# adityamwagh/SuperSLAM

Hardware: AMD Instinct MI355X
Metric: stereo pairs/sec (SPx2+LG) at 1376x376 (higher is better)
Workload: dtype f16; 1 GPU; configs[1]: SuperPoint x2 + select + gather + 1x LightGlue on 1376x376 stereo pairs; a step = 8 x 64 = 512 pairs per GPU resident in HBM (8 library calls of 64 pairs, different images per call), max_keypoints 600, seeded synthetic weights; pairs_per_call=64, max_keypoints=600, matches_last_call=1412, parallelism=replicated weights, pairs sharded over 1 rank(s), no data-path collective

## Files before the change

### superslam_amd/csrc/api.hip

```cpp
#include <algorithm>
#include <atomic>
#include <cmath>
#include <cstdarg>
#include <cstdlib>
#include <cstring>
#include <fstream>
#include <map>
#include <memory>
#include <mutex>
#include <string>
#include <vector>

#include "../../include/sship.h"
#include "../../include/superslam_hip/place_recognizer.hpp"
#include "kernels.h"
#include "stage_layout.h"

namespace sship {

static thread_local std::string g_err;
static void (*g_log_cb)(int, const char*) = nullptr;
static int g_profiling = 0;

void set_error(const std::string& msg) {
// ... 791 lines not shown
  KpRefineArgs r{};
  r.logits = sp->logits.as<float>(); r.img_stride = (size_t)Hc * Wc * kLogitStride; r.cell_stride = kLogitStride; r.chan_stride = 1;
  r.Hc = Hc; r.Wc = Wc; r.pix = sp->pix.as<int>(); r.n_dev = n_dev; r.n_host = 0; r.max_kp = sp->cfg.max_keypoints;
  r.kp_xys = kp; r.scale_x = scale_x; r.scale_y = scale_y; r.offsets = nullptr;
  launch_kp_refine(r, B, s);
  return hipGetLastError();
}
static int sp_select(sship_sp* sp, int B, int H, int W, float* scores_out, float* kp_out, int* n_out, hipStream_t s) {
  int H2, W2, H4, W4, Hc, Wc;
  sp_shapes(H, W, H2, W2, H4, W4, Hc, Wc);
  if (sp->cand_zero_ptr != sp->cand_count.p || sp->cand_zero_n < B || sp->cand_zero_stream != s)
    SSHIP_HIP_CHECK(hipMemsetAsync(sp->cand_count.p, 0, (size_t)B * 4, s));
  sp->cand_zero_ptr = sp->cand_count.p; sp->cand_zero_n = 0; sp->cand_zero_stream = s;
  NmsArgs a{};
  a.logits = sp->logits.as<float>(); a.ls = kLogitStride; a.B = B; a.H = Hc * 8; a.W = Wc * 8;
  a.radius = sp->cfg.nms_radius; a.thr_f = sp->thr_f; a.border = sp->cfg.remove_borders;
  a.cand = sp->cand.as<unsigned long long>(); a.cand_count = sp->cand_count.as<int>(); a.cap = sp->cap;
  a.scores_out = scores_out;
  launch_nms_tile(0, a, s);
  g_timer.mark_fine("sp_extract_stereo:select/nms_tile", s);
  TopkArgs t{};
  t.cand = a.cand; t.cand_count = a.cand_count; t.cap = sp->cap; t.max_kp = sp->cfg.max_keypoints;
  t.score_w = Wc * 8;
  t.scale_x = static_cast<float>(W) / (Wc * 8);
  t.scale_y = static_cast<float>(H) / (Hc * 8);
  t.desc_h = Hc; t.desc_w = Wc; t.kp_xys = kp_out; t.cell_h = sp->cell_h.as<int>(); t.cell_w = sp->cell_w.as<int>();
  t.n_out = n_out; t.n_cand_out = nullptr; t.reset_count = a.cand_count;
  t.pix = sp_wants_pix(sp) ? sp->pix.as<int>() : nullptr;
  launch_topk(t, B, s);
  SSHIP_HIP_CHECK(hipGetLastError());
  sp->cand_zero_n = B;
  if (sp->kp_refinement == SSHIP_KP_SUBPIXEL) {
    g_timer.mark_fine("sp_extract_stereo:select/topk", s);
    SSHIP_HIP_CHECK(sp_refine(sp, B, Hc, Wc, kp_out, n_out, t.scale_x, t.scale_y, s));
    g_timer.mark(g_profiling >= 2 ? "sp_extract_stereo:select/kp_refine" : "sp_extract_stereo:select", s);
    return SSHIP_OK;
  }
  g_timer.mark(g_profiling >= 2 ? "sp_extract_stereo:select/topk" : "sp_extract_stereo:select", s);
  return SSHIP_OK;
}

static hipError_t conv1ab(sship_sp* sp, const uint8_t* img, _Float16* out, int B, int H, int W, hipStream_t s) {
#if SSHIP_DEV_SWITCHES
  if (conv_mode() == 2) return sp_conv1ab_fused(sp->c1b, sp->w1a_frag, sp->b1a, img, out, B, H, W, s);
#endif
  return sp_conv1ab_pp(sp->c1b, sp->w1a_fragb, sp->b1a, img, out, B, H, W, s);
}

extern "C" int sship_sp_create(const sship_sp_config* cfg, sship_sp** out) {
  bind_thread();
  if (!cfg || !out || !cfg->weights_path) return fail(SSHIP_ERR_INVALID, "sp_create: null argument");
  if (cfg->max_keypoints <= 0 || cfg->max_keypoints > kMaxKp) return fail(SSHIP_ERR_INVALID, "sp_create: max_keypoints must be in [1, 4096]");
  if (cfg->nms_radius < 0 || cfg->nms_radius > 8) return fail(SSHIP_ERR_INVALID, "sp_create: nms_radius must be in [0, 8]");
  if (int rc = require_device()) return rc;
  StateDict sd; std::string err;
  if (!load_safetensors(cfg->weights_path, sd, err)) return fail(SSHIP_ERR_IO, err);
  std::unique_ptr<sship_sp, void (*)(sship_sp*)> sp(new sship_sp(), sship_sp_destroy);
  sp->cfg = *cfg;
  if (sp->cfg.pool_slots <= 0) sp->cfg.pool_slots = 8;
  if (sp->cfg.max_batch <= 0) sp->cfg.max_batch = 2;
  sp->cfg.weights_path = nullptr;
  sp->thr_f = threshold_as_float(cfg->keypoint_threshold);
  struct L { const char* name; int cout, cin, ks, ct; ConvW* dst; };
  const L layers[] = {{"conv1b", 64, 64, 3, 64, &sp->c1b}, {"conv2a", 64, 64, 3, 64, &sp->c2a},
                      {"conv2b", 64, 64, 3, 64, &sp->c2b}, {"conv3a", 128, 64, 3, 64, &sp->c3a},
                      {"conv3b", 128, 128, 3, 32, &sp->c3b}, {"conv4a", 128, 128, 3, 32, &sp->c4a},
                      {"conv4b", 128, 128, 3, 32, &sp->c4b}, {"convPa", 256, 128, 3, 32, &sp->cPa},
                      {"convPb", 65, 256, 1, 96, &sp->cPb}, {"convDa", 256, 128, 3, 32, &sp->cDa},
                      {"convDb", 256, 256, 1, 128, &sp->cDb}};
  for (const L& l : layers) {
    const Tensor* w = find_tensor(sd, std::string(l.name) + ".weight", {l.cout, l.cin, l.ks, l.ks}, err);
    const Tensor* b = w ? find_tensor(sd, std::string(l.name) + ".bias", {l.cout}, err) : nullptr;
    if (!w || !b) return fail(SSHIP_ERR_IO, err);
    if (int rc = upload_conv(w->data.data(), b->data.data(), l.cout, l.cin, l.ks, l.ct, *l.dst)) return rc;
    if (l.ks == 3 && std::string(l.name) != "convDa" && std::string(l.name) != "conv1b")
      if (int rc = upload_conv_q(w->data.data(), l.cout, l.cin, *l.dst)) return rc;
#if SSHIP_DEV_SWITCHES
    if (std::string(l.name) == "conv2a" || std::string(l.name) == "conv2b")
      if (int rc = upload_wino(w->data.data(), *l.dst)) return rc;
#endif
    if (std::string(l.name) == "convDb")
      if (int rc = upload_conv(w->data.data(), b->data.data(), l.cout, l.cin, 1, 32, sp->cDb32)) return rc;
    if (std::string(l.name) == "convPb") {
      std::vector<_Float16> plain((size_t)80 * 256, (_Float16)0.f);
      for (int co = 0; co < 65; ++co)
        for (int ci = 0; ci < 256; ++ci) plain[(size_t)co * 256 + ci] = (_Float16)w->data[(size_t)co * 256 + ci];
      SSHIP_HIP_CHECK(hipMalloc(reinterpret_cast<void**>(&l.dst->w_q), plain.size() * sizeof(_Float16)));
      SSHIP_HIP_CHECK(hipMemcpy(l.dst->w_q, plain.data(), plain.size() * sizeof(_Float16), hipMemcpyHostToDevice));
    }
  }
  {
    const Tensor* w = find_tensor(sd, "conv1a.weight", {64, 1, 3, 3}, err);
    const Tensor* b = w ? find_tensor(sd, "conv1a.bias", {64}, err) : nullptr;
    if (!w || !b) return fail(SSHIP_ERR_IO, err);
    std::vector<float> wt(576);
    for (int co = 0; co < 64; ++co)
      for (int t = 0; t < 9; ++t) wt[t * 64 + co] = (float)(_Float16)w->data[co * 9 + t];
    if (int rc = upload_floats(wt.data(), 576, &sp->w1a)) return rc;
    if (int rc = upload_floats(b->data.data(), 64, &sp->b1a)) return rc;
    std::vector<_Float16> fr(2 * 64 * 8);
    for (int mt = 0; mt < 2; ++mt)
      for (int lane = 0; lane < 64; ++lane)
        for (int e = 0; e < 8; ++e) {
          const int co = mt * 32 + (lane & 31), k = (lane >> 5) * 8 + e;
          fr[(mt * 64 + lane) * 8 + e] = (_Float16)(k < 9 ? w->data[co * 9 + k] : 0.f);
        }
    SSHIP_HIP_CHECK(hipMalloc(reinterpret_cast<void**>(&sp->w1a_frag), fr.size() * sizeof(_Float16)));
    SSHIP_HIP_CHECK(hipMemcpy(sp->w1a_frag, fr.data(), fr.size() * sizeof(_Float16), hipMemcpyHostToDevice));
    std::fill(fr.begin(), fr.end(), (_Float16)0.f);
    for (int mt = 0; mt < 2; ++mt)
      for (int lane = 0; lane < 64; ++lane) {
        const int co = mt * 32 + (lane & 31), hh = lane >> 5;
        _Float16* f = &fr[(mt * 64 + lane) * 8];
        if (hh == 0) {
          for (int e = 0; e < 5; ++e) f[e] = (_Float16)w->data[co * 9 + e];
        } else {
          for (int e = 0; e < 4; ++e) f[e] = (_Float16)w->data[co * 9 + 5 + e];
          const _Float16 hi = (_Float16)b->data[co];
          f[4] = hi;
          f[5] = (_Float16)(b->data[co] - (float)hi);
        }
      }
    SSHIP_HIP_CHECK(hipMalloc(reinterpret_cast<void**>(&sp->w1a_fragb), fr.size() * sizeof(_Float16)));
    SSHIP_HIP_CHECK(hipMemcpy(sp->w1a_fragb, fr.data(), fr.size() * sizeof(_Float16), hipMemcpyHostToDevice));
  }
  SSHIP_HIP_CHECK(hipStreamCreateWithFlags(&sp->stream, hipStreamDefault));
  if (int rc = sship_pool_create(sp->cfg.pool_slots, sp->cfg.max_keypoints, SSHIP_DESC_DIM, &sp->pool)) return rc;
  *out = sp.release();
  return SSHIP_OK;
}
extern "C" void sship_sp_destroy(sship_sp* sp) {
  bind_thread();
  if (!sp) return;
  (void)hipDeviceSynchronize();
  for (ConvW* c : {&sp->c1b, &sp->c2a, &sp->c2b, &sp->c3a, &sp->c3b, &sp->c4a, &sp->c4b, &sp->cPa, &sp->cPb, &sp->cDa, &sp->cDb, &sp->cDb32})
    free_conv(*c);
  if (sp->w1a) (void)hipFree(sp->w1a);
  if (sp->b1a) (void)hipFree(sp->b1a);
  if (sp->w1a_frag) (void)hipFree(sp->w1a_frag);
  if (sp->w1a_fragb) (void)hipFree(sp->w1a_fragb);
  ring_free(sp);
  if (sp->pool) sship_pool_destroy(sp->pool);
  sp->pool = nullptr;
  if (sp->stream) (void)hipStreamDestroy(sp->stream);
  delete sp;
}
extern "C" int sship_sp_debug_activation(sship_sp* sp, int layer, void* out_host, unsigned long long bytes) {
  bind_thread();
  if (!sp || !out_host) return fail(SSHIP_ERR_INVALID, "sp_debug_activation: null argument");
  DevBuf* bufs[12] = {nullptr, &sp->a1b, &sp->a2a, &sp->a2b, &sp->a3a, &sp->a3b, &sp->a4a, &sp->a4b, &sp->aPa, &sp->aDa, &sp->draw, &sp->logits};
  if (layer < 1 || layer > 11 || !bufs[layer]->p || bytes > bufs[layer]->bytes) return fail(SSHIP_ERR_INVALID, "sp_debug_activation: bad layer / size");
  SSHIP_HIP_CHECK(hipDeviceSynchronize());
  SSHIP_HIP_CHECK(hipMemcpy(out_host, bufs[layer]->p, bytes, hipMemcpyDeviceToHost));
  return SSHIP_OK;
}
extern "C" sship_pool* sship_sp_pool(sship_sp* sp) {
  bind_thread(); return sp ? sp->pool : nullptr; }
extern "C" int sship_sp_max_keypoints(const sship_sp* sp) { return sp ? sp->cfg.max_keypoints : 0; }
extern "C" int sship_sp_set_descriptor_sampling(sship_sp* sp, int mode) {
  if (!sp) return fail(SSHIP_ERR_INVALID, "sp_set_descriptor_sampling: null handle");
  if (mode != SSHIP_DESC_NEAREST && mode != SSHIP_DESC_BILINEAR)
    return fail(SSHIP_ERR_INVALID, "sp_set_descriptor_sampling: mode must be 0 (nearest) or 1 (bilinear)");
  for (const auto& pd : sp->ring.pending)
    if (pd.active) return fail(SSHIP_ERR_INVALID, "sp_set_descriptor_sampling: a ring submission is pending (collect it with sship_sp_extract_stereo_ring first)");
#if SSHIP_DEV_SWITCHES
  if (mode == SSHIP_DESC_BILINEAR && desc_dense_mode()) return fail(SSHIP_ERR_INVALID, "sp_set_descriptor_sampling: bilinear sampling is not available under SUPERSLAM_HIP_DESC=dense");
#endif
  sp->desc_sampling = mode;
  return SSHIP_OK;
}
extern "C" int sship_sp_descriptor_sampling(const sship_sp* sp) { return sp ? sp->desc_sampling : SSHIP_DESC_NEAREST; }
extern "C" int sship_sp_set_keypoint_refinement(sship_sp* sp, int mode) {
  if (!sp) return fail(SSHIP_ERR_INVALID, "sp_set_keypoint_refinement: null handle");
  if (mode != SSHIP_KP_INTEGER && mode != SSHIP_KP_SUBPIXEL)
    return fail(SSHIP_ERR_INVALID, "sp_set_keypoint_refinement: mode must be 0 (integer) or 1 (sub-pixel)");
  for (const auto& pd : sp->ring.pending)
    if (pd.active) return fail(SSHIP_ERR_INVALID, "sp_set_keypoint_refinement: a ring submission is pending (collect it with sship_sp_extract_stereo_ring first)");
  sp->kp_refinement = mode;
  return SSHIP_OK;
}
extern "C" int sship_sp_keypoint_refinement(const sship_sp* sp) { return sp ? sp->kp_refinement : SSHIP_KP_INTEGER; }

extern "C" int sship_sp_extract_batch_device(sship_sp* sp, const uint8_t* imgs, int batch, int h, int w, void* desc_out,
                                             float* kp_out, int* n_out, void* stream) {
  bind_thread();
  if (!sp || !imgs || !desc_out || !kp_out || !n_out || batch <= 0) return fail(SSHIP_ERR_INVALID, "sp_extract_batch_device: bad arguments");
  hipStream_t s = static_cast<hipStream_t>(stream);
  if (int rc = sp_ensure(sp, batch, h, w)) return rc;
  if (g_profiling && imgs != sp->img.as<uint8_t>())
    SSHIP_HIP_CHECK(hipMemcpyAsync(sp->img.p, imgs, (size_t)batch * h * w, hipMemcpyDeviceToDevice, s));
  sp->img_valid = g_profiling != 0 || imgs == sp->img.as<uint8_t>();
  g_timer.begin(s);
  if (int rc = sp_network(sp, imgs, batch, h, w, s, false)) return rc;
  if (int rc = sp_select(sp, batch, h, w, nullptr, kp_out, n_out, s)) return rc;
  int H2, W2, H4, W4, Hc, Wc;
  sp_shapes(h, w, H2, W2, H4, W4, Hc, Wc);
  SSHIP_HIP_CHECK(desc_head(sp, 0, Hc, Wc, sp->cell_h.as<int>(), sp->cell_w.as<int>(), n_out, batch, static_cast<_Float16*>(desc_out),
                            (size_t)sp->cfg.max_keypoints * 256, s));
  g_timer.mark("sp_extract_stereo:gather", s);
  return SSHIP_OK;
}

extern "C" int sship_sp_dense(sship_sp* sp, const uint8_t* imgs, int batch, int h, int w, float* scores, void* desc_grid,
                              float* logits, void* stream) {
  bind_thread();
  if (!sp || !imgs || batch <= 0) return fail(SSHIP_ERR_INVALID, "sp_dense: bad arguments");
  hipStream_t s = static_cast<hipStream_t>(stream);
  if (int rc = sp_ensure(sp, batch, h, w)) return rc;
  if (int rc = sp_network(sp, imgs, batch, h, w, s, desc_grid != nullptr)) return rc;
  int H2, W2, H4, W4, Hc, Wc;
  sp_shapes(h, w, H2, W2, H4, W4, Hc, Wc);
  if (scores) {
    NmsArgs a{};
    a.logits = sp->logits.as<float>(); a.ls = kLogitStride; a.B = batch; a.H = Hc * 8; a.W = Wc * 8;
    a.radius = sp->cfg.nms_radius; a.scores_out = scores;
    launch_nms_tile(0, a, s);
  }
  if (desc_grid) launch_desc_dense_chw(sp->draw.as<_Float16>(), Hc * Wc, batch, static_cast<_Float16*>(desc_grid), s);
  if (logits) launch_logits_chw(sp->logits.as<float>(), kLogitStride, Hc * Wc, batch, logits, s);
  SSHIP_HIP_CHECK(hipGetLastError());
  return SSHIP_OK;
}

extern "C" int sship_mfma_probe(int random_operands, float* tflops) {
  bind_thread();
  if (!tflops) return fail(SSHIP_ERR_INVALID, "mfma_probe: null argument");
  if (int rc = require_device()) return rc;
  SSHIP_HIP_CHECK(mfma_probe(random_operands != 0, tflops));
  return SSHIP_OK;
}

extern "C" int sship_sp_bench_layer(sship_sp* sp, int layer, int batch, int h, int w, int iters, float* avg_ms,
                                    double* macs) {
  bind_thread();
  if (!sp || !avg_ms || iters <= 0 || layer < 0 || layer > 16) return fail(SSHIP_ERR_INVALID, "sp_bench_layer: bad arguments");
  if (batch > sp->wsB || h != sp->wsH || w != sp->wsW) return fail(SSHIP_ERR_INVALID, "sp_bench_layer: run the network at this shape first");
  if (layer <= 1 && !sp->img_valid)
    return fail(SSHIP_ERR_INVALID, "sp_bench_layer: the handle holds no copy of the last input - make one call with sship_set_profiling(1) first "
                                   "(a launch on stale / zero pixels runs at a higher clock than the real one)");
  int H2, W2, H4, W4, Hc, Wc;
  sp_shapes(h, w, H2, W2, H4, W4, Hc, Wc);
  hipStream_t s = sp->stream;
  _Float16 *a1a = sp->a1a.as<_Float16>(), *a1b = sp->a1b.as<_Float16>(), *a2a = sp->a2a.as<_Float16>(),
           *a2b = sp->a2b.as<_Float16>(), *a3a = sp->a3a.as<_Float16>(), *a3b = sp->a3b.as<_Float16>(),
           *a4a = sp->a4a.as<_Float16>(), *a4b = sp->a4b.as<_Float16>(), *aPa = sp->aPa.as<_Float16>(),
           *aDa = sp->aDa.as<_Float16>();
  const bool for_refine = layer == 16;
  auto run = [&]() -> hipError_t {
    switch (layer) {
      case 0: launch_conv1a(sp->img.as<uint8_t>(), sp->w1a, sp->b1a, a1a, batch, h, w, s); return hipGetLastError();
      case 1: return conv1ab(sp, sp->img.as<uint8_t>(), a1b, batch, h, w, s);
      case 15:
        if (!sp_conv2ab_fused_fits(batch, H2, W2, true)) return hipErrorInvalidValue;
        return sp_conv2ab_fused(sp->c2a, sp->c2b, a1b, a2b, batch, H2, W2, s);
      case 2: return conv3(sp->c2a, a1b, a2a, batch, H2, W2, false, s);
      case 3: return conv3(sp->c2b, a2a, a2b, batch, H2, W2, true, s);
      case 4: return conv3a_layer(sp->c3a, a2b, a3a, batch, H4, W4, s);
      case 5: return conv3(sp->c3b, a3a, a3b, batch, H4, W4, true, s);
      case 6: return conv3(sp->c4a, a3b, a4a, batch, Hc, Wc, false, s);
      case 7: return conv3(sp->c4b, a4a, a4b, batch, Hc, Wc, false, s);
      case 8: return conv3(sp->cPa, a4b, aPa, batch, Hc, Wc, false, s);
      case 9: return sp_conv1x1_f32(sp->cPb, aPa, sp->logits.as<float>(), kLogitStride, batch, Hc, Wc, s);
      case 10: return conv3(sp->cDa, a4b, aDa, batch, Hc, Wc, false, s);
      case 11: return sp_conv1x1_f16(sp->cDb, aDa, sp->draw.as<_Float16>(), batch, Hc, Wc, s);
      case 12: {
        if (hipError_t e = hipMemsetAsync(sp->cand_count.p, 0, (size_t)batch * 4, s)) return e;
        sp->cand_zero_n = 0;
        NmsArgs a{};
        a.logits = sp->logits.as<float>(); a.ls = kLogitStride; a.B = batch; a.H = Hc * 8; a.W = Wc * 8;
        a.radius = sp->cfg.nms_radius; a.thr_f = sp->thr_f; a.border = sp->cfg.remove_borders;
        a.cand = sp->cand.as<unsigned long long>(); a.cand_count = sp->cand_count.as<int>(); a.cap = sp->cap;
        launch_nms_tile(0, a, s);
        return hipGetLastError();
      }
      case 13: {
        TopkArgs t{};
        t.cand = sp->cand.as<unsigned long long>(); t.cand_count = sp->cand_count.as<int>(); t.cap = sp->cap;
        t.max_kp = sp->cfg.max_keypoints; t.score_w = Wc * 8;
        t.scale_x = static_cast<float>(w) / (Wc * 8); t.scale_y = static_cast<float>(h) / (Hc * 8);
        t.desc_h = Hc; t.desc_w = Wc; t.kp_xys = sp->kp.as<float>(); t.cell_h = sp->cell_h.as<int>(); t.cell_w = sp->cell_w.as<int>();
        t.n_out = sp->n_dev.as<int>(); t.n_cand_out = nullptr;
        t.pix = (sp_wants_pix(sp) || for_refine) ? sp->pix.as<int>() : nullptr;
        launch_topk(t, batch, s);
        return hipGetLastError();
      }
      case 16:
        return sp_refine(sp, batch, Hc, Wc, sp->kp.as<float>(), sp->n_dev.as<int>(), static_cast<float>(w) / (Wc * 8), static_cast<float>(h) / (Hc * 8), s);
      default:
        if (hipError_t e = sp->desc_stage.ensure((size_t)batch * sp->cfg.max_keypoints * 512)) return e;
        return desc_head(sp, 0, Hc, Wc, sp->cell_h.as<int>(), sp->cell_w.as<int>(), sp->n_dev.as<int>(), batch, sp->desc_stage.as<_Float16>(),
                         (size_t)sp->cfg.max_keypoints * 256, s);
    }
  };
  if (layer == 13 || layer == 14 || layer == 16) {
    const int keep = layer;
    layer = 12; SSHIP_HIP_CHECK(run());
    layer = 13; SSHIP_HIP_CHECK(run());
    layer = keep;
  }
  const double px[12] = {(double)h * w, (double)h * w, (double)H2 * W2, (double)H2 * W2, (double)H4 * W4, (double)H4 * W4,
                         (double)Hc * Wc, (double)Hc * Wc, (double)Hc * Wc, (double)Hc * Wc, (double)Hc * Wc, (double)Hc * Wc};
  const double mpp[12] = {9.0 * 64, 576.0 * 64 + 9.0 * 64 , 576.0 * 64, 576.0 * 64, 576.0 * 128, 1152.0 * 128, 1152.0 * 128,
                          1152.0 * 128, 1152.0 * 256, 256.0 * 65, 1152.0 * 256, 256.0 * 256};
  if (macs) *macs = layer < 12 ? px[layer] * mpp[layer] * batch : layer == 15 ? (px[2] * mpp[2] + px[3] * mpp[3]) * batch : 0.0;
  return bench_loop(s, iters, run, avg_ms);
}
// ... 2590 lines not shown
```

### superslam_amd/csrc/sp_convs.hip

```cpp
#include <cstdlib>
#include <string>

#include "igemm.h"
#include "kernels.h"

namespace sship {

static IgemmArgs conv_args(const ConvW& w, const _Float16* in, int B, int H, int W) {
  IgemmArgs a{};
  a.in0 = in; a.in1 = in; a.cin0 = w.cin; a.cs0 = w.cin; a.cs1 = w.cin;
  a.wpack = w.w; a.bias = w.bias; a.B = B; a.H = H; a.W = W; a.cout = w.cout; a.ostride = w.cout;
  return a;
}

hipError_t sp_conv1x1_f16(const ConvW& w, const _Float16* in, _Float16* out, int B, int H, int W, hipStream_t s) {
  IgemmArgs a = conv_args(w, in, B, H, W);
  a.out0 = out;
  if (w.cin != 256) return hipErrorInvalidValue;
  return launch_igemm<1, 256, 128, 4, EpiF16<false, false>>(a, w.cout_pad, s);
}

typedef float f4x_t __attribute__((ext_vector_type(4)));
__global__ __launch_bounds__(256, 2) void k_convpb_stream(const _Float16* __restrict__ in, const _Float16* __restrict__ w,
                                                          const float* __restrict__ bias, float* __restrict__ out, int P,
                                                          int ostride) {
  __shared__ __attribute__((aligned(16))) _Float16 s_a4[8 * 512];
  const int lane = threadIdx.x & 63, n = lane & 15, kb = lane >> 4;
  for (int u = threadIdx.x; u < 8 * 64; u += 256) {
    const int ks = u >> 6, l = u & 63;
    *reinterpret_cast<uint4*>(s_a4 + u * 8) = *reinterpret_cast<const uint4*>(w + (size_t)(64 + (l & 15)) * 256 + ks * 32 + (l >> 4) * 8);
  }
  h8_t a[4][8];
#pragma unroll
  for (int m = 0; m < 4; ++m)
#pragma unroll
    for (int ks = 0; ks < 8; ++ks) a[m][ks] = *reinterpret_cast<const h8_t*>(w + (size_t)(16 * m + n) * 256 + ks * 32 + kb * 8);
  __shared__ __attribute__((aligned(16))) float s_b[80];
  if (threadIdx.x < 80) s_b[threadIdx.x] = threadIdx.x < 65 ? bias[threadIdx.x] : 0.f;
  __syncthreads();
  const int ntiles = (P + 15) >> 4, nwaves = gridDim.x * 4;
  const _Float16* src = in + kb * 8;
  h8_t fA[8], fB[8];
  auto fetch = [&](h8_t (&f)[8], int t) __attribute__((always_inline)) {
    const int pix = min(min(t, ntiles - 1) * 16 + n, P - 1);
    const _Float16* p = src + (size_t)pix * 256;
#pragma unroll
    for (int ks = 0; ks < 8; ++ks) f[ks] = *reinterpret_cast<const h8_t*>(p + ks * 32);
  };
  auto tile = [&](const h8_t (&f)[8], int t) __attribute__((always_inline)) {
    f4x_t acc[5];
#pragma unroll
    for (int m = 0; m < 5; ++m) acc[m] = *reinterpret_cast<const f4x_t*>(s_b + 16 * m + 4 * kb);
#pragma unroll
    for (int ks = 0; ks < 8; ++ks) {
      const h8_t a4 = *reinterpret_cast<const h8_t*>(s_a4 + (ks * 64 + lane) * 8);
#pragma unroll
      for (int m = 0; m < 4; ++m) acc[m] = __builtin_amdgcn_mfma_f32_16x16x32_f16(a[m][ks], f[ks], acc[m], 0, 0, 0);
      acc[4] = __builtin_amdgcn_mfma_f32_16x16x32_f16(a4, f[ks], acc[4], 0, 0, 0);
    }
    const int pix = t * 16 + n;
    if (pix < P) {
      float* o = out + (size_t)pix * ostride + 4 * kb;
#pragma unroll
      for (int m = 0; m < 4; ++m) *reinterpret_cast<f4x_t*>(o + 16 * m) = acc[m];
      if (kb == 0) o[64] = acc[4][0];
    }
  };
  const int t0 = blockIdx.x * 4 + (threadIdx.x >> 6);
  fetch(fA, t0);
  for (int t = t0; t < ntiles; t += 2 * nwaves) {
    fetch(fB, t + nwaves);
    __builtin_amdgcn_sched_barrier(0);
    tile(fA, t);
    if (t + nwaves < ntiles) {
      fetch(fA, t + 2 * nwaves);
      __builtin_amdgcn_sched_barrier(0);
      tile(fB, t + nwaves);
    }
  }
}

hipError_t sp_conv1x1_f32(const ConvW& w, const _Float16* in, float* out, int ostride, int B, int H, int W,
                          hipStream_t s) {
  if (w.cin != 256) return hipErrorInvalidValue;
  static const bool use_igemm = dev_env("SUPERSLAM_HIP_CONVPB") && std::string(dev_env("SUPERSLAM_HIP_CONVPB")) == "igemm";
  if (w.w_q && w.cout == 65 && ostride >= 68 && ostride % 4 == 0 && !use_igemm) {
    const int P = B * H * W;
    int wgs = 2 * cu_count();
    if (wgs * 4 > (P + 15) / 16) wgs = ((P + 15) / 16 + 3) / 4;
    hipLaunchKernelGGL(k_convpb_stream, dim3(wgs), dim3(256), 0, s, in, w.w_q, w.bias, out, P, ostride);
    return hipGetLastError();
  }
#if SSHIP_DEV_SWITCHES
  IgemmArgs a = conv_args(w, in, B, H, W);
  a.out0 = out; a.ostride = ostride;
  return launch_igemm<1, 256, 96, 4, EpiF32>(a, w.cout_pad, s);
#else
  return hipErrorInvalidValue;
#endif
}

constexpr int kDhLd = 264;
__global__ __launch_bounds__(512) void k_desc_head_gather(const _Float16* __restrict__ da, int Hc, int Wc,
                                                          const int* __restrict__ cell_h, const int* __restrict__ cell_w,
                                                          const int* __restrict__ n_dev, int max_kp,
                                                          const _Float16* __restrict__ wp, const float* __restrict__ bias,
                                                          _Float16* __restrict__ out, size_t out_img_stride) {
  __shared__ __attribute__((aligned(16))) _Float16 s_x[64 * kDhLd];
  __shared__ float s_red[8][64];
  const int b = blockIdx.y, i0 = blockIdx.x * 64;
  const int n = n_dev[b];
  if (i0 >= n) return;
  const int tid = threadIdx.x, wave = tid >> 6, lane = tid & 63, j = lane & 31, hh = lane >> 5;
  const _Float16* img = da + (size_t)b * Hc * Wc * 256;
  for (int u = tid; u < 64 * 32; u += 512) {
    const int r = u >> 5, part = u & 31;
    uint4 v = make_uint4(0, 0, 0, 0);
    if (i0 + r < n) {
      const int ch = cell_h[(size_t)b * max_kp + i0 + r], cw = cell_w[(size_t)b * max_kp + i0 + r];
      v = *reinterpret_cast<const uint4*>(img + ((size_t)ch * Wc + cw) * 256 + part * 8);
    }
    *reinterpret_cast<uint4*>(s_x + r * kDhLd + part * 8) = v;
  }
  h8_t a[16];
  {
    const _Float16* w = wp + (size_t)wave * (16 * 512) + lane * 8;
#pragma unroll
    for (int ks = 0; ks < 16; ++ks) a[ks] = *reinterpret_cast<const h8_t*>(w + ks * 512);
  }
  __syncthreads();
  f16x_t acc[2];
#pragma unroll
  for (int nn = 0; nn < 2; ++nn)
#pragma unroll
    for (int r = 0; r < 16; ++r) acc[nn][r] = 0.f;
#pragma unroll
  for (int ks = 0; ks < 16; ++ks) {
    const h8_t b0 = *reinterpret_cast<const h8_t*>(s_x + j * kDhLd + ks * 16 + hh * 8);
    const h8_t b1 = *reinterpret_cast<const h8_t*>(s_x + (32 + j) * kDhLd + ks * 16 + hh * 8);
    acc[0] = mfma32(a[ks], b0, acc[0]);
    acc[1] = mfma32(a[ks], b1, acc[1]);
  }
  float v[2][16];
#pragma unroll
  for (int g = 0; g < 4; ++g) {
    const float4 bv = *reinterpret_cast<const float4*>(bias + wave * 32 + hh * 4 + g * 8);
    const float bb[4] = {bv.x, bv.y, bv.z, bv.w};
#pragma unroll
    for (int nn = 0; nn < 2; ++nn)
#pragma unroll
      for (int e = 0; e < 4; ++e) v[nn][4 * g + e] = (float)(_Float16)(acc[nn][4 * g + e] + bb[e]);
  }
  auto row_sum_sq = [&](float (&tot)[2]) {
#pragma unroll
    for (int nn = 0; nn < 2; ++nn) {
      float ss = 0.f;
#pragma unroll
      for (int r = 0; r < 16; ++r) ss += v[nn][r] * v[nn][r];
      ss += __shfl_xor(ss, 32, 64);
      if (hh == 0) s_red[wave][nn * 32 + j] = ss;
    }
    __syncthreads();
#pragma unroll
    for (int nn = 0; nn < 2; ++nn) {
      float t = 0.f;
#pragma unroll
      for (int w = 0; w < 8; ++w) t += s_red[w][nn * 32 + j];
      tot[nn] = t;
    }
    __syncthreads();
  };
  float tot[2];
  row_sum_sq(tot);
#pragma unroll
  for (int nn = 0; nn < 2; ++nn) {
    const float denom = fmaxf(sqrtf(tot[nn]), 1e-12f);
#pragma unroll
    for (int r = 0; r < 16; ++r) v[nn][r] = (float)(_Float16)(v[nn][r] / denom);
  }
  row_sum_sq(tot);
#pragma unroll
  for (int nn = 0; nn < 2; ++nn) {
    const int i = i0 + nn * 32 + j;
    if (i >= n) continue;
    const float inv = rsqrtf(tot[nn] + 1e-12f);
    _Float16* orow = out + (size_t)b * out_img_stride + (size_t)i * 256 + wave * 32 + hh * 4;
#pragma unroll
    for (int g = 0; g < 4; ++g)
      *reinterpret_cast<h4_t*>(orow + g * 8) =
          to_h4(v[nn][4 * g] * inv, v[nn][4 * g + 1] * inv, v[nn][4 * g + 2] * inv, v[nn][4 * g + 3] * inv);
  }
}

constexpr int kDsPatchLd = 584;
template <int NN, bool BIL = false>
__global__ __launch_bounds__(512) void k_desc_head_sparse(const _Float16* __restrict__ a4b, int Hc, int Wc,
                                                          const int* __restrict__ cell_h, const int* __restrict__ cell_w,
                                                          const int* __restrict__ n_dev, int max_kp,
                                                          const _Float16* __restrict__ wda, const float* __restrict__ bda,
                                                          const _Float16* __restrict__ wdb, const float* __restrict__ bdb,
                                                          _Float16* __restrict__ out, size_t out_img_stride) {
  extern __shared__ __attribute__((aligned(16))) char ds_smem[];
  _Float16* s_p = reinterpret_cast<_Float16*>(ds_smem);
  constexpr int NK = 32 * NN;
  _Float16* s_x = s_p + NK * kDsPatchLd;
  float (*s_red)[64] = reinterpret_cast<float (*)[64]>(s_x + NK * kDhLd);
  int* s_cell = reinterpret_cast<int*>(s_red + 8);
  float* s_wt = reinterpret_cast<float*>(s_cell + 64);
  const int b = blockIdx.y, i0 = blockIdx.x * (BIL ? NK / 4 : NK);
  const int n = min(max(n_dev[b], 0), max_kp);
  if (i0 >= n) return;
  const int tid = threadIdx.x, wave = tid >> 6, lane = tid & 63, j = lane & 31, hh = lane >> 5;
  if constexpr (BIL) {
    if (tid < NK) {
      const int i = i0 + (tid >> 2), q = tid & 3;
      int c = -1;
      float wq = 0.f;
      if (i < n) {
        const int px = cell_h[(size_t)b * max_kp + i];
        int x0, y0;
        float fx, fy;
        bilinear_corner((float)(px & 0xffff), (float)(px >> 16), Hc, Wc, x0, y0, fx, fy);
        const int cy = y0 + (q >> 1), cx = x0 + (q & 1);
        if (cy >= 0 && cy < Hc && cx >= 0 && cx < Wc) { c = (cy << 16) | cx; wq = bilinear_weight(q, fx, fy); }
      }
      s_cell[tid] = c;
      s_wt[tid] = wq;
    }
  } else {
    if (tid < NK)
      s_cell[tid] = i0 + tid < n ? (cell_h[(size_t)b * max_kp + i0 + tid] << 16) | cell_w[(size_t)b * max_kp + i0 + tid] : -1;
  }
  const _Float16* img = a4b + (size_t)b * Hc * Wc * 128;
  f16x_t acc[NN];
#pragma unroll
  for (int g = 0; g < 4; ++g) {
    const float4 bv = *reinterpret_cast<const float4*>(bda + wave * 32 + hh * 4 + g * 8);
#pragma unroll
    for (int nn = 0; nn < NN; ++nn) { acc[nn][4 * g] = bv.x; acc[nn][4 * g + 1] = bv.y; acc[nn][4 * g + 2] = bv.z; acc[nn][4 * g + 3] = bv.w; }
  }
  const _Float16* wa = wda + (size_t)wave * (72 * 512) + lane * 8;
  auto frag_of = [](int idx, int& tap, int& ks) __attribute__((always_inline)) {
    const int h32 = idx / 18, r18 = idx - 18 * h32, t6 = r18 / 3, ky = r18 - 3 * t6;
    tap = ky * 3 + (t6 >> 1); ks = 2 * h32 + (t6 & 1);
  };
  auto wfrag = [&](int lin) __attribute__((always_inline)) {
    int tap, ks;
    frag_of(lin % 36, tap, ks);
    return *reinterpret_cast<const h8_t*>(wa + (((lin / 36) * 9 + tap) * 4 + ks) * 512);
  };
  h8_t fa[2][12];
#pragma unroll
  for (int i = 0; i < 12; ++i) fa[0][i] = wfrag(i);
  __syncthreads();
#pragma unroll
  for (int chunk = 0; chunk < 2; ++chunk) {
    if (chunk) __syncthreads();
    for (int u = tid; u < NK * 72; u += 512) {
      const int kp = u / 72, rem = u - kp * 72, tap = rem >> 3, part = rem & 7;
      const int ky = tap / 3, kx = tap - ky * 3;
      const int c = s_cell[kp];
      const int y = (c >> 16) + ky - 1, x = (c & 0xffff) + kx - 1;
      uint4 v = make_uint4(0, 0, 0, 0);
      if (c >= 0 && y >= 0 && y < Hc && x >= 0 && x < Wc)
        v = *reinterpret_cast<const uint4*>(img + ((size_t)y * Wc + x) * 128 + chunk * 64 + part * 8);
      *reinterpret_cast<uint4*>(s_p + kp * kDsPatchLd + tap * 64 + part * 8) = v;
    }
    __syncthreads();
#pragma unroll
    for (int grp = 0; grp < 3; ++grp) {
      const int g_lin = chunk * 3 + grp;
      if (g_lin + 1 < 6) {
#pragma unroll
        for (int i = 0; i < 12; ++i) fa[(g_lin + 1) & 1][i] = wfrag((g_lin + 1) * 12 + i);
      }
      __builtin_amdgcn_sched_barrier(0);
#pragma unroll
      for (int i = 0; i < 12; ++i) {
        int tap, ks;
        frag_of(grp * 12 + i, tap, ks);
#pragma unroll
        for (int nn = 0; nn < NN; ++nn) {
          const h8_t bf = *reinterpret_cast<const h8_t*>(s_p + (nn * 32 + j) * kDsPatchLd + tap * 64 + ks * 16 + hh * 8);
          acc[nn] = mfma32(fa[g_lin & 1][i], bf, acc[nn]);
        }
      }
    }
  }
  h8_t a[16];
  {
    const _Float16* w = wdb + (size_t)wave * (16 * 512) + lane * 8;
#pragma unroll
    for (int ks = 0; ks < 16; ++ks) a[ks] = *reinterpret_cast<const h8_t*>(w + ks * 512);
  }
#pragma unroll
  for (int g = 0; g < 4; ++g) {
#pragma unroll
    for (int nn = 0; nn < NN; ++nn)
      *reinterpret_cast<h4_t*>(s_x + (nn * 32 + j) * kDhLd + wave * 32 + hh * 4 + g * 8) =
          to_h4(fmaxf(acc[nn][4 * g], 0.f), fmaxf(acc[nn][4 * g + 1], 0.f), fmaxf(acc[nn][4 * g + 2], 0.f), fmaxf(acc[nn][4 * g + 3], 0.f));
  }
  __syncthreads();
#pragma unroll
  for (int nn = 0; nn < NN; ++nn)
#pragma unroll
    for (int r = 0; r < 16; ++r) acc[nn][r] = 0.f;
#pragma unroll
  for (int ks = 0; ks < 16; ++ks) {
#pragma unroll
    for (int nn = 0; nn < NN; ++nn) {
      const h8_t bf = *reinterpret_cast<const h8_t*>(s_x + (nn * 32 + j) * kDhLd + ks * 16 + hh * 8);
      acc[nn] = mfma32(a[ks], bf, acc[nn]);
    }
  }
  float v[NN][16];
#pragma unroll
  for (int g = 0; g < 4; ++g) {
    const float4 bv = *reinterpret_cast<const float4*>(bdb + wave * 32 + hh * 4 + g * 8);
    const float bb[4] = {bv.x, bv.y, bv.z, bv.w};
#pragma unroll
    for (int nn = 0; nn < NN; ++nn)
#pragma unroll
      for (int e = 0; e < 4; ++e) v[nn][4 * g + e] = (float)(_Float16)(acc[nn][4 * g + e] + bb[e]);
  }
  auto row_sum_sq = [&](float (&tot)[NN]) {
#pragma unroll
    for (int nn = 0; nn < NN; ++nn) {
      float ss = 0.f;
#pragma unroll
      for (int r = 0; r < 16; ++r) ss += v[nn][r] * v[nn][r];
      ss += __shfl_xor(ss, 32, 64);
      if (hh == 0) s_red[wave][nn * 32 + j] = ss;
    }
    __syncthreads();
#pragma unroll
    for (int nn = 0; nn < NN; ++nn) {
      float t = 0.f;
#pragma unroll
      for (int w = 0; w < 8; ++w) t += s_red[w][nn * 32 + j];
      tot[nn] = t;
    }
    __syncthreads();
  };
  float tot[NN];
  row_sum_sq(tot);
#pragma unroll
  for (int nn = 0; nn < NN; ++nn) {
    const float denom = fmaxf(sqrtf(tot[nn]), 1e-12f);
#pragma unroll
    for (int r = 0; r < 16; ++r) v[nn][r] = (float)(_Float16)(v[nn][r] / denom);
  }
  if constexpr (BIL) {
#pragma unroll
    for (int nn = 0; nn < NN; ++nn) {
      const float wq = s_wt[nn * 32 + j];
#pragma unroll
      for (int r = 0; r < 16; ++r) {
        float t = v[nn][r] * wq;
        t += __shfl_xor(t, 1, 64);
        t += __shfl_xor(t, 2, 64);
        v[nn][r] = t;
      }
    }
    row_sum_sq(tot);
#pragma unroll
    for (int nn = 0; nn < NN; ++nn) {
      const int i = i0 + ((nn * 32 + j) >> 2), q = j & 3;
      if (i >= n) continue;
      const float denom = fmaxf(sqrtf(tot[nn]), 1e-12f);
      _Float16* orow = out + (size_t)b * out_img_stride + (size_t)i * 256 + wave * 32 + hh * 4;
#pragma unroll
      for (int g = 0; g < 4; ++g)
        if (q == g)
          *reinterpret_cast<h4_t*>(orow + g * 8) =
              to_h4(v[nn][4 * g] / denom, v[nn][4 * g + 1] / denom, v[nn][4 * g + 2] / denom, v[nn][4 * g + 3] / denom);
    }
    return;
  }
  row_sum_sq(tot);
#pragma unroll
  for (int nn = 0; nn < NN; ++nn) {
    const int i = i0 + nn * 32 + j;
    if (i >= n) continue;
    const float inv = rsqrtf(tot[nn] + 1e-12f);
    _Float16* orow = out + (size_t)b * out_img_stride + (size_t)i * 256 + wave * 32 + hh * 4;
#pragma unroll
    for (int g = 0; g < 4; ++g)
      *reinterpret_cast<h4_t*>(orow + g * 8) =
          to_h4(v[nn][4 * g] * inv, v[nn][4 * g + 1] * inv, v[nn][4 * g + 2] * inv, v[nn][4 * g + 3] * inv);
  }
}

hipError_t launch_desc_head_sparse_bilinear(const ConvW& da32, const ConvW& db32, const _Float16* a4b, int Hc, int Wc, const int* pix,
                                            const int* n_dev, int max_kp, int B, _Float16* out, size_t out_img_stride, hipStream_t s) {
  if (da32.cin != 128 || da32.cout != 256 || da32.ct != 32 || da32.ks != 3) return hipErrorInvalidValue;
  if (Hc > 4095 || Wc > 8191) return hipErrorInvalidValue;
  constexpr size_t smem = (size_t)64 * kDsPatchLd * 2 + (size_t)64 * kDhLd * 2 + 8 * 64 * 4 + 64 * 4 + 64 * 4;
  static const hipError_t attr_rc = [] {
    hipError_t e = hipFuncSetAttribute(reinterpret_cast<const void*>(k_desc_head_sparse<2, true>), hipFuncAttributeMaxDynamicSharedMemorySize, (int)smem);
    if (e != hipSuccess) return e;
    return hipFuncSetAttribute(reinterpret_cast<const void*>(k_desc_head_sparse<1, true>), hipFuncAttributeMaxDynamicSharedMemorySize, (int)smem);
  }();
  if (attr_rc != hipSuccess) return attr_rc;
  if (B * ((max_kp + 15) / 16) * 2 <= cu_count())
    hipLaunchKernelGGL((k_desc_head_sparse<1, true>), dim3((max_kp + 7) / 8, B), dim3(512), smem, s, a4b, Hc, Wc, pix, nullptr, n_dev,
                       max_kp, da32.w, da32.bias, db32.w, db32.bias, out, out_img_stride);
  else
    hipLaunchKernelGGL((k_desc_head_sparse<2, true>), dim3((max_kp + 15) / 16, B), dim3(512), smem, s, a4b, Hc, Wc, pix, nullptr, n_dev,
                       max_kp, da32.w, da32.bias, db32.w, db32.bias, out, out_img_stride);
  return hipGetLastError();
}

hipError_t launch_desc_head_sparse(const ConvW& da32, const ConvW& db32, const _Float16* a4b, int Hc, int Wc, const int* cell_h,
                                   const int* cell_w, const int* n_dev, int max_kp, int B, _Float16* out, size_t out_img_stride,
                                   hipStream_t s) {
  if (da32.cin != 128 || da32.cout != 256 || da32.ct != 32 || da32.ks != 3) return hipErrorInvalidValue;
  constexpr size_t smem = (size_t)64 * kDsPatchLd * 2 + (size_t)64 * kDhLd * 2 + 8 * 64 * 4 + 64 * 4;
  static const hipError_t attr_rc = [] {
    hipError_t e = hipFuncSetAttribute(reinterpret_cast<const void*>(k_desc_head_sparse<2>), hipFuncAttributeMaxDynamicSharedMemorySize, (int)smem);
    if (e != hipSuccess) return e;
    return hipFuncSetAttribute(reinterpret_cast<const void*>(k_desc_head_sparse<1>), hipFuncAttributeMaxDynamicSharedMemorySize, (int)smem);
  }();
  if (attr_rc != hipSuccess) return attr_rc;
  if (B * ((max_kp + 63) / 64) * 2 <= cu_count())
    hipLaunchKernelGGL(k_desc_head_sparse<1>, dim3((max_kp + 31) / 32, B), dim3(512), smem, s, a4b, Hc, Wc, cell_h, cell_w, n_dev,
                       max_kp, da32.w, da32.bias, db32.w, db32.bias, out, out_img_stride);
  else
    hipLaunchKernelGGL(k_desc_head_sparse<2>, dim3((max_kp + 63) / 64, B), dim3(512), smem, s, a4b, Hc, Wc, cell_h, cell_w, n_dev,
                       max_kp, da32.w, da32.bias, db32.w, db32.bias, out, out_img_stride);
  return hipGetLastError();
}

void launch_desc_head_gather(const ConvW& db32, const _Float16* da, int Hc, int Wc, const int* cell_h, const int* cell_w,
                             const int* n_dev, int max_kp, int B, _Float16* out, size_t out_img_stride, hipStream_t s) {
  hipLaunchKernelGGL(k_desc_head_gather, dim3((max_kp + 63) / 64, B), dim3(512), 0, s, da, Hc, Wc, cell_h, cell_w, n_dev,
                     max_kp, db32.w, db32.bias, out, out_img_stride);
}

}
```

Baseline: 5631 pairs/s.

## Coalesce convPb logit stores via LDS and add async-DMA two-WG descriptor head

The 65-channel logit conv now stages each wave's 16-pixel output tile in LDS and writes it back as contiguous 16-byte chunks, instead of strided per-pixel stores. This only works when ostride is 68. The sparse descriptor head gets a new kernel for the multi-block case. It double-buffers the 3x3 patch gathers through buffer_load ... lds direct-to-LDS DMA, prefetches weight fragments, and uses a smaller LDS footprint so two workgroups can share a CU. The shared tail is factored into a helper, and debug entry points are added, at the cost of inline-asm complexity and a new size limit on the input buffer.

After: 5687 pairs/s, median of 6. +1.0%, better.

```diff
diff --git a/superslam_amd/csrc/api.hip b/superslam_amd/csrc/api.hip
--- a/superslam_amd/csrc/api.hip
+++ b/superslam_amd/csrc/api.hip
@@ -967,6 +967,23 @@
   if (layer < 1 || layer > 11 || !bufs[layer]->p || bytes > bufs[layer]->bytes) return fail(SSHIP_ERR_INVALID, "sp_debug_activation: bad layer / size");
   SSHIP_HIP_CHECK(hipDeviceSynchronize());
   SSHIP_HIP_CHECK(hipMemcpy(out_host, bufs[layer]->p, bytes, hipMemcpyDeviceToHost));
+  return SSHIP_OK;
+}
+extern "C" int sship_sp_debug_convpb(sship_sp* sp, const void* in_fp16_dev, int pixels, float* logits_dev) {
+  bind_thread();
+  if (!sp || !in_fp16_dev || !logits_dev || pixels <= 0) return fail(SSHIP_ERR_INVALID, "sp_debug_convpb: bad arguments");
+  SSHIP_HIP_CHECK(sp_conv1x1_f32(sp->cPb, static_cast<const _Float16*>(in_fp16_dev), logits_dev, kLogitStride, 1, 1, pixels, sp->stream));
+  SSHIP_HIP_CHECK(hipStreamSynchronize(sp->stream));
+  return SSHIP_OK;
+}
+extern "C" int sship_sp_debug_desc_head(sship_sp* sp, const void* a4b_fp16_dev, int batch, int Hc, int Wc, const int* cell_h_dev,
+                                        const int* cell_w_dev, const int* n_dev, int max_kp, void* desc_fp16_dev) {
+  bind_thread();
+  if (!sp || !a4b_fp16_dev || !cell_h_dev || !cell_w_dev || !n_dev || !desc_fp16_dev || batch <= 0 || Hc <= 0 || Wc <= 0 || max_kp <= 0)
+    return fail(SSHIP_ERR_INVALID, "sp_debug_desc_head: bad arguments");
+  SSHIP_HIP_CHECK(launch_desc_head_sparse(sp->cDa, sp->cDb32, static_cast<const _Float16*>(a4b_fp16_dev), Hc, Wc, cell_h_dev, cell_w_dev, n_dev,
+                                          max_kp, batch, static_cast<_Float16*>(desc_fp16_dev), (size_t)max_kp * 256, sp->stream));
+  SSHIP_HIP_CHECK(hipStreamSynchronize(sp->stream));
   return SSHIP_OK;
 }
 extern "C" sship_pool* sship_sp_pool(sship_sp* sp) {
diff --git a/superslam_amd/csrc/sp_convs.hip b/superslam_amd/csrc/sp_convs.hip
--- a/superslam_amd/csrc/sp_convs.hip
+++ b/superslam_amd/csrc/sp_convs.hip
@@ -21,6 +21,12 @@
 }
 
 typedef float f4x_t __attribute__((ext_vector_type(4)));
+__device__ __forceinline__ void wave_lds_sync() {
+  __builtin_amdgcn_fence(__ATOMIC_RELEASE, "wavefront");
+  __builtin_amdgcn_wave_barrier();
+  __builtin_amdgcn_fence(__ATOMIC_ACQUIRE, "wavefront");
+}
+template <bool WHOLE>
 __global__ __launch_bounds__(256, 2) void k_convpb_stream(const _Float16* __restrict__ in, const _Float16* __restrict__ w,
                                                           const float* __restrict__ bias, float* __restrict__ out, int P,
                                                           int ostride) {
@@ -37,6 +43,8 @@
     for (int ks = 0; ks < 8; ++ks) a[m][ks] = *reinterpret_cast<const h8_t*>(w + (size_t)(16 * m + n) * 256 + ks * 32 + kb * 8);
   __shared__ __attribute__((aligned(16))) float s_b[80];
   if (threadIdx.x < 80) s_b[threadIdx.x] = threadIdx.x < 65 ? bias[threadIdx.x] : 0.f;
+  __shared__ __attribute__((aligned(16))) float s_o[WHOLE ? 4 * 16 * 68 : 4];
+  float* patch = s_o + (WHOLE ? (threadIdx.x >> 6) * (16 * 68) : 0);
   __syncthreads();
   const int ntiles = (P + 15) >> 4, nwaves = gridDim.x * 4;
   const _Float16* src = in + kb * 8;
@@ -58,12 +66,27 @@
       for (int m = 0; m < 4; ++m) acc[m] = __builtin_amdgcn_mfma_f32_16x16x32_f16(a[m][ks], f[ks], acc[m], 0, 0, 0);
       acc[4] = __builtin_amdgcn_mfma_f32_16x16x32_f16(a4, f[ks], acc[4], 0, 0, 0);
     }
-    const int pix = t * 16 + n;
-    if (pix < P) {
-      float* o = out + (size_t)pix * ostride + 4 * kb;
-#pragma unroll
-      for (int m = 0; m < 4; ++m) *reinterpret_cast<f4x_t*>(o + 16 * m) = acc[m];
-      if (kb == 0) o[64] = acc[4][0];
+    if constexpr (WHOLE) {
+      wave_lds_sync();
+#pragma unroll
+      for (int m = 0; m < 4; ++m) *reinterpret_cast<f4x_t*>(patch + n * 68 + 16 * m + 4 * kb) = acc[m];
+      if (kb == 0) *reinterpret_cast<f4x_t*>(patch + n * 68 + 64) = f4x_t{acc[4][0], 0.f, 0.f, 0.f};
+      wave_lds_sync();
+      const int units = 17 * min(16, P - t * 16);
+      float* o = out + (size_t)t * (16 * 68);
+#pragma unroll
+      for (int i = 0; i < 5; ++i) {
+        const int u = i * 64 + lane;
+        if (u < units) *reinterpret_cast<f4x_t*>(o + 4 * u) = *reinterpret_cast<const f4x_t*>(patch + 4 * u);
+      }
+    } else {
+      const int pix = t * 16 + n;
+      if (pix < P) {
+        float* o = out + (size_t)pix * ostride + 4 * kb;
+#pragma unroll
+        for (int m = 0; m < 4; ++m) *reinterpret_cast<f4x_t*>(o + 16 * m) = acc[m];
+        if (kb == 0) o[64] = acc[4][0];
+      }
     }
   };
   const int t0 = blockIdx.x * 4 + (threadIdx.x >> 6);
@@ -88,7 +111,15 @@
     const int P = B * H * W;
     int wgs = 2 * cu_count();
     if (wgs * 4 > (P + 15) / 16) wgs = ((P + 15) / 16 + 3) / 4;
-    hipLaunchKernelGGL(k_convpb_stream, dim3(wgs), dim3(256), 0, s, in, w.w_q, w.bias, out, P, ostride);
+#if SSHIP_DEV_SWITCHES
+    static const bool pieces = dev_env("SUPERSLAM_HIP_CONVPB") && std::string(dev_env("SUPERSLAM_HIP_CONVPB")) == "pieces";
+    if (pieces) {
+      hipLaunchKernelGGL(k_convpb_stream<false>, dim3(wgs), dim3(256), 0, s, in, w.w_q, w.bias, out, P, ostride);
+      return hipGetLastError();
+    }
+#endif
+    if (ostride != 68) return hipErrorInvalidValue;
+    hipLaunchKernelGGL(k_convpb_stream<true>, dim3(wgs), dim3(256), 0, s, in, w.w_q, w.bias, out, P, ostride);
     return hipGetLastError();
   }
 #if SSHIP_DEV_SWITCHES
@@ -193,6 +224,10 @@
 }
 
 constexpr int kDsPatchLd = 584;
+template <int NN, bool BIL>
+__device__ __forceinline__ void desc_head_tail(f16x_t (&acc)[NN], _Float16* s_x, float (*s_red)[64], const float* s_wt,
+                                               const _Float16* __restrict__ wdb, const float* __restrict__ bdb,
+                                               _Float16* __restrict__ out_img, int i0, int n);
 template <int NN, bool BIL = false>
 __global__ __launch_bounds__(512) void k_desc_head_sparse(const _Float16* __restrict__ a4b, int Hc, int Wc,
                                                           const int* __restrict__ cell_h, const int* __restrict__ cell_w,
@@ -287,6 +322,14 @@
       }
     }
   }
+  desc_head_tail<NN, BIL>(acc, s_x, s_red, s_wt, wdb, bdb, out + (size_t)b * out_img_stride, i0, n);
+}
+
+template <int NN, bool BIL>
+__device__ __forceinline__ void desc_head_tail(f16x_t (&acc)[NN], _Float16* s_x, float (*s_red)[64], const float* s_wt,
+                                               const _Float16* __restrict__ wdb, const float* __restrict__ bdb,
+                                               _Float16* __restrict__ out_img, int i0, int n) {
+  const int tid = threadIdx.x, wave = tid >> 6, lane = tid & 63, j = lane & 31, hh = lane >> 5;
   h8_t a[16];
   {
     const _Float16* w = wdb + (size_t)wave * (16 * 512) + lane * 8;
@@ -368,7 +411,7 @@
       const int i = i0 + ((nn * 32 + j) >> 2), q = j & 3;
       if (i >= n) continue;
       const float denom = fmaxf(sqrtf(tot[nn]), 1e-12f);
-      _Float16* orow = out + (size_t)b * out_img_stride + (size_t)i * 256 + wave * 32 + hh * 4;
+      _Float16* orow = out_img + (size_t)i * 256 + wave * 32 + hh * 4;
 #pragma unroll
       for (int g = 0; g < 4; ++g)
         if (q == g)
@@ -383,12 +426,108 @@
     const int i = i0 + nn * 32 + j;
     if (i >= n) continue;
     const float inv = rsqrtf(tot[nn] + 1e-12f);
-    _Float16* orow = out + (size_t)b * out_img_stride + (size_t)i * 256 + wave * 32 + hh * 4;
+    _Float16* orow = out_img + (size_t)i * 256 + wave * 32 + hh * 4;
 #pragma unroll
     for (int g = 0; g < 4; ++g)
       *reinterpret_cast<h4_t*>(orow + g * 8) =
           to_h4(v[nn][4 * g] * inv, v[nn][4 * g + 1] * inv, v[nn][4 * g + 2] * inv, v[nn][4 * g + 3] * inv);
   }
+}
+
+constexpr int kDqLd = 296;
+constexpr int kDqBufBytes = 64 * kDqLd * 2;
+constexpr unsigned kDqOob = 0x80000000u;
+constexpr size_t kDqSmem = 2 * (size_t)kDqBufBytes + 8 * 64 * 4 + 64 * 4;
+static_assert(kDqBufBytes == 37 * 1024 && 64 * kDhLd * 2 <= kDqBufBytes && 2 * kDqSmem <= 160 * 1024, "descriptor head LDS layout");
+__global__ __launch_bounds__(512, 4) void k_desc_head_sparse_2wg(const _Float16* __restrict__ a4b, int Hc, int Wc,
+                                                                 const int* __restrict__ cell_h, const int* __restrict__ cell_w,
+                                                                 const int* __restrict__ n_dev, int max_kp,
+                                                                 const _Float16* __restrict__ wda, const float* __restrict__ bda,
+                                                                 const _Float16* __restrict__ wdb, const float* __restrict__ bdb,
+                                                                 _Float16* __restrict__ out, size_t out_img_stride) {
+  extern __shared__ __attribute__((aligned(16))) char ds_smem[];
+  _Float16* s_p = reinterpret_cast<_Float16*>(ds_smem);
+  float (*s_red)[64] = reinterpret_cast<float (*)[64]>(ds_smem + 2 * kDqBufBytes);
+  int* s_cell = reinterpret_cast<int*>(s_red + 8);
+  const int b = blockIdx.y, i0 = blockIdx.x * 64;
+  const int n = min(max(n_dev[b], 0), max_kp);
+  if (i0 >= n) return;
+  const int tid = threadIdx.x, wave = __builtin_amdgcn_readfirstlane(tid >> 6), lane = tid & 63, j = lane & 31, hh = lane >> 5;
+  if (tid < 64)
+    s_cell[tid] = i0 + tid < n ? (cell_h[(size_t)b * max_kp + i0 + tid] << 16) | cell_w[(size_t)b * max_kp + i0 + tid] : -1;
+  f16x_t acc[2];
+#pragma unroll
+  for (int g = 0; g < 4; ++g) {
+    const float4 bv = *reinterpret_cast<const float4*>(bda + wave * 32 + hh * 4 + g * 8);
+#pragma unroll
+    for (int nn = 0; nn < 2; ++nn) { acc[nn][4 * g] = bv.x; acc[nn][4 * g + 1] = bv.y; acc[nn][4 * g + 2] = bv.z; acc[nn][4 * g + 3] = bv.w; }
+  }
+  const _Float16* wa = wda + (size_t)wave * (72 * 512) + lane * 8;
+  auto wfrag = [&](int q, int r18) __attribute__((always_inline)) {
+    const int t6 = r18 / 3, ky = r18 - 3 * t6, tap = ky * 3 + (t6 >> 1), ks = 2 * (q & 1) + (t6 & 1);
+    return *reinterpret_cast<const h8_t*>(wa + (((q >> 1) * 9 + tap) * 4 + ks) * 512);
+  };
+  h8_t fa[2][6];
+#pragma unroll
+  for (int i = 0; i < 6; ++i) fa[0][i] = wfrag(0, i);
+  typedef int rsrc4_t __attribute__((ext_vector_type(4)));
+  rsrc4_t rs;
+  {
+    const unsigned long long ba = (unsigned long long)(uintptr_t)(a4b + (size_t)b * Hc * Wc * 128);
+    rs[0] = __builtin_amdgcn_readfirstlane((int)(unsigned)ba);
+    rs[1] = __builtin_amdgcn_readfirstlane((int)((unsigned)(ba >> 32) & 0xffffu));
+    rs[2] = __builtin_amdgcn_readfirstlane(Hc * Wc * 256);
+    rs[3] = 0x00020000;
+  }
+  __syncthreads();
+  unsigned voff[5];
+#pragma unroll
+  for (int k = 0; k < 5; ++k) {
+    const int slot = (wave + 8 * k) * 64 + lane, kp = min(slot / 37, 63), within = slot - (slot / 37) * 37;
+    const int tap = within >> 2, ky = tap / 3, kx = tap - ky * 3;
+    const int c = s_cell[kp];
+    const int y = (c >> 16) + ky - 1, x = (c & 0xffff) + kx - 1;
+    const bool ok = within < 36 && c >= 0 && y >= 0 && y < Hc && x >= 0 && x < Wc;
+    voff[k] = ok ? (unsigned)(y * Wc + x) * 256u + (unsigned)(within & 3) * 16u : kDqOob;
+  }
+  const unsigned lds0 = __builtin_amdgcn_readfirstlane((unsigned)(uintptr_t)s_p);
+  auto dma = [&](int q) __attribute__((always_inline)) {
+#pragma unroll
+    for (int k = 0; k < 5; ++k) {
+      if (wave + 8 * k >= 37) continue;
+      const unsigned dst = lds0 + (unsigned)((q & 1) * kDqBufBytes + (wave + 8 * k) * 1024), v = voff[k] + 64u * q;
+      unsigned keep;
+      asm volatile("s_mov_b32 %0, m0\n\ts_mov_b32 m0, %2\n\ts_nop 0\n\tbuffer_load_dwordx4 %1, %3, 0 offen lds\n\ts_mov_b32 m0, %0"
+                   : "=&s"(keep) : "v"(v), "s"(dst), "s"(rs) : "memory");
+    }
+  };
+  dma(0);
+#pragma unroll
+  for (int q = 0; q < 4; ++q) {
+    asm volatile("s_waitcnt vmcnt(0)" ::: "memory");
+    __syncthreads();
+    const _Float16* sq = s_p + (q & 1) * (64 * kDqLd);
+#pragma unroll
+    for (int grp = 0; grp < 3; ++grp) {
+      const int g_lin = q * 3 + grp;
+      if (g_lin + 1 < 12) {
+#pragma unroll
+        for (int i = 0; i < 6; ++i) fa[(g_lin + 1) & 1][i] = wfrag((g_lin + 1) / 3, ((g_lin + 1) % 3) * 6 + i);
+      }
+      if (grp == 0 && q < 3) dma(q + 1);
+      __builtin_amdgcn_sched_barrier(0);
+#pragma unroll
+      for (int i = 0; i < 6; ++i) {
+        const int r18 = grp * 6 + i, t6 = r18 / 3, ky = r18 - 3 * t6, tap = ky * 3 + (t6 >> 1);
+#pragma unroll
+        for (int nn = 0; nn < 2; ++nn) {
+          const h8_t bf = *reinterpret_cast<const h8_t*>(sq + (nn * 32 + j) * kDqLd + tap * 32 + (t6 & 1) * 16 + hh * 8);
+          acc[nn] = mfma32(fa[g_lin & 1][i], bf, acc[nn]);
+        }
+      }
+    }
+  }
+  desc_head_tail<2, false>(acc, s_p, s_red, nullptr, wdb, bdb, out + (size_t)b * out_img_stride, i0, n);
 }
 
 hipError_t launch_desc_head_sparse_bilinear(const ConvW& da32, const ConvW& db32, const _Float16* a4b, int Hc, int Wc, const int* pix,
@@ -417,17 +556,31 @@
   if (da32.cin != 128 || da32.cout != 256 || da32.ct != 32 || da32.ks != 3) return hipErrorInvalidValue;
   constexpr size_t smem = (size_t)64 * kDsPatchLd * 2 + (size_t)64 * kDhLd * 2 + 8 * 64 * 4 + 64 * 4;
   static const hipError_t attr_rc = [] {
-    hipError_t e = hipFuncSetAttribute(reinterpret_cast<const void*>(k_desc_head_sparse<2>), hipFuncAttributeMaxDynamicSharedMemorySize, (int)smem);
+    hipError_t e = hipFuncSetAttribute(reinterpret_cast<const void*>(k_desc_head_sparse_2wg), hipFuncAttributeMaxDynamicSharedMemorySize, (int)kDqSmem);
     if (e != hipSuccess) return e;
+#if SSHIP_DEV_SWITCHES
+    e = hipFuncSetAttribute(reinterpret_cast<const void*>(k_desc_head_sparse<2>), hipFuncAttributeMaxDynamicSharedMemorySize, (int)smem);
+    if (e != hipSuccess) return e;
+#endif
     return hipFuncSetAttribute(reinterpret_cast<const void*>(k_desc_head_sparse<1>), hipFuncAttributeMaxDynamicSharedMemorySize, (int)smem);
   }();
   if (attr_rc != hipSuccess) return attr_rc;
-  if (B * ((max_kp + 63) / 64) * 2 <= cu_count())
+  static const std::string form = [] { const char* e = dev_env("SUPERSLAM_HIP_DESC_HEAD"); return std::string(e ? e : ""); }();
+  if (B * ((max_kp + 63) / 64) * 2 <= cu_count() && form != "1wg" && form != "2wg") {
     hipLaunchKernelGGL(k_desc_head_sparse<1>, dim3((max_kp + 31) / 32, B), dim3(512), smem, s, a4b, Hc, Wc, cell_h, cell_w, n_dev,
                        max_kp, da32.w, da32.bias, db32.w, db32.bias, out, out_img_stride);
-  else
+    return hipGetLastError();
+  }
+#if SSHIP_DEV_SWITCHES
+  if (form == "1wg") {
     hipLaunchKernelGGL(k_desc_head_sparse<2>, dim3((max_kp + 63) / 64, B), dim3(512), smem, s, a4b, Hc, Wc, cell_h, cell_w, n_dev,
                        max_kp, da32.w, da32.bias, db32.w, db32.bias, out, out_img_stride);
+    return hipGetLastError();
+  }
+#endif
+  if ((long long)Hc * Wc * 256 >= (1ll << 31)) return hipErrorInvalidValue;
+  hipLaunchKernelGGL(k_desc_head_sparse_2wg, dim3((max_kp + 63) / 64, B), dim3(512), kDqSmem, s, a4b, Hc, Wc, cell_h, cell_w, n_dev,
+                     max_kp, da32.w, da32.bias, db32.w, db32.bias, out, out_img_stride);
   return hipGetLastError();
 }
 
```
